# isarandi/metrabs

Hardware: NVIDIA H100
Metric: crops/sec (higher is better)
Workload: dtype bf16

## Files before the change

metrabs_b200/csrc/tc_fmb.cuh:

```cuda
#pragma once
#include "tc_gemm.cuh"

namespace mtb {

constexpr int FMB_NC = 128;
constexpr int FMB_BOX_H = TC_TILE_H + 2;
constexpr int FMB_BOX_BYTES = TC_TILE_W * FMB_BOX_H * TC_BK * 2;
constexpr int FMB_W_BYTES = FMB_NC * TC_BK * 2;
constexpr int FMB_A2_BYTES = TC_BM * FMB_NC * 2;

template <int BN2>
struct FmbSmem {
  static constexpr int kchunks = BN2 == 128 ? 2 : 1;
  static constexpr int stages = BN2 == 128 ? 4 : 8;
  static constexpr int ring_off = 3 * kchunks * FMB_BOX_BYTES;
  static constexpr int a2_off = ring_off + stages * FMB_W_BYTES;
  static constexpr int bar_off = a2_off + FMB_A2_BYTES;
  static constexpr int smem_bytes = bar_off + 256 + 1024 ;
};

struct FmbParams {
  TcConvParams g;
  const float* bias1;
  int Cexp, nch, has_res;
};

template <typename T, int BN2>
__global__ void __launch_bounds__(TC_THREADS, 1)
fmb_kernel(const __grid_constant__ CUtensorMap tmA, const __grid_constant__ CUtensorMap tmW1, const __grid_constant__ CUtensorMap tmW2,
           const FmbParams p) {
  using L = FmbSmem<BN2>;
  constexpr int STAGES = L::stages, KCH = L::kchunks, NUM_KB = 9 * KCH;
  extern __shared__ uint8_t tc_smem_raw[];
  uint8_t* smem = (uint8_t*)(((uintptr_t)tc_smem_raw + 1023) & ~(uintptr_t)1023);
  uint64_t* full = (uint64_t*)(smem + L::bar_off);
  uint64_t* empty = full + STAGES;
  uint64_t* box_full = empty + STAGES;
  uint64_t* box_empty = box_full + 1;
  const TcConvParams& g = p.g;

  const int warp = threadIdx.x >> 5, lane = threadIdx.x & 31;
  if (threadIdx.x == TC_CONSUMER_WARPS * 32) {
    tma_prefetch_desc(&tmA);
    tma_prefetch_desc(&tmW1);
    tma_prefetch_desc(&tmW2);
    for (int i = 0; i < STAGES; ++i) {
      mbar_init(&full[i], 1);
      mbar_init(&empty[i], TC_CONSUMER_WARPS);
    }
    mbar_init(box_full, 1);
    mbar_init(box_empty, TC_CONSUMER_WARPS);
    fence_barrier_init();
  }
  __syncthreads();

  if (warp == TC_CONSUMER_WARPS) {
    if (lane == 0) {
      int it = 0, n = 0;
      for (int t = blockIdx.x; t < g.m_tiles; t += gridDim.x, ++n) {
        mbar_wait(box_empty, (n & 1) ^ 1);
        mbar_expect_tx(box_full, 3 * KCH * FMB_BOX_BYTES);
#pragma unroll
        for (int kc = 0; kc < KCH; ++kc) tma_load_tap_boxes(smem + 3 * kc * FMB_BOX_BYTES, FMB_BOX_BYTES, &tmA, box_full, g, t, kc);
        for (int c = 0; c < p.nch; ++c) {
          for (int kb = 0; kb < NUM_KB + 2; ++kb, ++it) {
            const int s = it % STAGES;
            mbar_wait(&empty[s], ((it / STAGES) & 1) ^ 1);
            uint8_t* st = smem + L::ring_off + s * FMB_W_BYTES;
            if (kb < NUM_KB) {
              const int tap = kb / KCH, kc = kb - tap * KCH;
              mbar_expect_tx(&full[s], FMB_W_BYTES);
              tma_load_2d(st, &tmW1, &full[s], tap * g.Cin + kc * TC_BK, c * FMB_NC);
            } else {
              mbar_expect_tx(&full[s], BN2 * TC_BK * 2);
              tma_load_2d(st, &tmW2, &full[s], c * FMB_NC + (kb - NUM_KB) * TC_BK, 0);
            }
          }
        }
      }
    }
    return;
  }
  const int wg = warp >> 2;
  const uint32_t boxes = smem_u32(smem) + wg * 64 * 128, ring = smem_u32(smem + L::ring_off), a2 = smem_u32(smem + L::a2_off);
  const int r0 = wg * 64 + (warp & 3) * 16 + (lane >> 2);
  typedef typename Pair16<T>::type T2;
  const T* __restrict__ res = (const T*)g.res;
  T* __restrict__ out = (T*)g.out;
  int it = 0, n = 0;
  for (int t = blockIdx.x; t < g.m_tiles; t += gridDim.x, ++n) {
    float acc2[BN2 / 2];
#pragma unroll
    for (int i = 0; i < BN2 / 2; ++i) acc2[i] = 0.f;
    mbar_wait(box_full, n & 1);
    for (int c = 0; c < p.nch; ++c) {
      float acc1[FMB_NC / 2];
#pragma unroll
      for (int i = 0; i < FMB_NC / 2; ++i) acc1[i] = 0.f;
      int prev = -1;
      for (int kb = 0; kb < NUM_KB; ++kb, ++it) {
        const int s = it % STAGES;
        mbar_wait(&full[s], (it / STAGES) & 1);
        const int tap = kb / KCH, kc = kb - tap * KCH, r = tap / 3, sx = tap - 3 * r;
        const uint32_t a = boxes + (uint32_t)(3 * kc + sx) * FMB_BOX_BYTES + (uint32_t)r * (TC_TILE_W * 128);
        const uint32_t b = ring + s * FMB_W_BYTES;
        wgmma_fence();
#pragma unroll
        for (int k = 0; k < TC_BK / 16; ++k)
          wgmma_16b<T, FMB_NC>(acc1, gmma_desc<128>(a + 32 * k), gmma_desc<128>(b + 32 * k), (uint32_t)(kb | k));
        wgmma_commit();
        wgmma_wait<1>();
        if (prev >= 0) {
          __syncwarp();
          if (lane == 0) mbar_arrive(&empty[prev]);
        }
        prev = s;
      }
      wgmma_wait<0>();
      wgmma_fence_regs<FMB_NC / 2>(acc1);
      __syncwarp();
      if (lane == 0) {
        mbar_arrive(&empty[prev]);
        if (c == p.nch - 1) mbar_arrive(box_empty);
      }
#pragma unroll
      for (int j = 0; j < FMB_NC / 8; ++j) {
        const int cc = 8 * j + 2 * (lane & 3);
        const int col = c * FMB_NC + cc;
        float2 bv = make_float2(0.f, 0.f);
        if (col < p.Cexp) bv = __ldg(reinterpret_cast<const float2*>(p.bias1 + col));
        const uint32_t sub = (uint32_t)(cc >> 6) * (TC_BM * 128), kc = (uint32_t)(cc & 63);
#pragma unroll
        for (int h = 0; h < 2; ++h) {
          const int r = r0 + 8 * h;
          T2 v = Pair16<T>::pack(0.f, 0.f);
          if (col < p.Cexp)
            v = Pair16<T>::pack(tc_act<ACT_SILU, T>(acc1[4 * j + 2 * h] + bv.x), tc_act<ACT_SILU, T>(acc1[4 * j + 2 * h + 1] + bv.y));
          const uint32_t off = sub + (uint32_t)r * 128 + ((((kc >> 3) ^ (uint32_t)(r & 7))) << 4) + (kc & 7) * 2;
          *reinterpret_cast<T2*>(smem + L::a2_off + off) = v;
        }
      }
      fence_proxy_async();
      wg_sync(wg);
      {
        const int s0 = it % STAGES, s1 = (it + 1) % STAGES;
        mbar_wait(&full[s0], (it / STAGES) & 1);
        mbar_wait(&full[s1], ((it + 1) / STAGES) & 1);
        wgmma_fence();
#pragma unroll
        for (int k = 0; k < FMB_NC / 16; ++k) {
          const uint32_t sub = (uint32_t)(k >> 2), ko = (uint32_t)(k & 3) * 32;
          const uint32_t b = ring + (sub ? s1 : s0) * FMB_W_BYTES;
          wgmma_16b<T, BN2>(acc2, gmma_desc<128>(a2 + sub * (TC_BM * 128) + wg * 64 * 128 + ko), gmma_desc<128>(b + ko), (uint32_t)(c | k));
        }
        wgmma_commit();
        wgmma_wait<0>();
        wgmma_fence_regs<BN2 / 2>(acc2);
        __syncwarp();
        if (lane == 0) {
          mbar_arrive(&empty[s0]);
          mbar_arrive(&empty[s1]);
        }
        it += 2;
      }
    }
    const int c0 = 2 * (lane & 3);
#pragma unroll
    for (int h = 0; h < 2; ++h) {
      size_t off;
      if (!tile_row_offset(1, t, r0 + 8 * h, g.M, g.Cout, g.tiles_w, g.tiles_h, g.Hout, g.Wout, off)) continue;
#pragma unroll
      for (int j = 0; j < BN2 / 8; ++j) {
        const int cidx = c0 + 8 * j;
        if (cidx >= g.Cout) break;
        const float2 bv = __ldg(reinterpret_cast<const float2*>(g.bias + cidx));
        float o0 = acc2[4 * j + 2 * h] + bv.x, o1 = acc2[4 * j + 2 * h + 1] + bv.y;
        if (p.has_res) {
          const float2 rv = Pair16<T>::unpack(*reinterpret_cast<const T2*>(res + off + cidx));
          o0 += rv.x;
          o1 += rv.y;
        }
        *reinterpret_cast<T2*>(out + off + cidx) = Pair16<T>::pack(o0, o1);
      }
    }
  }
}

struct FmbWeights {
  bool ready = false;
  const TcWeights* w1 = nullptr;
  const TcWeights* w2 = nullptr;
  int Cin = 0, Cexp = 0, Cout = 0, bn2 = 0;
  mutable TmapCache maps;
};

inline bool fmb_shape_ok(int cin, int cexp, int cout) {
  return cin % 16 == 0 && cin >= 16 && cin <= 96 && cout == cin && cexp % 16 == 0 && cexp >= 32 && cexp <= 512;
}

inline void fmb_prepare(FmbWeights& f, const TcWeights& w1, const TcWeights& w2) {
  f.ready = false;
  if (!fmb_shape_ok(w1.Cin, w1.Cout, w2.Cout) || w2.Cin != w1.Cout || w1.taps != 9) return;
  f.w1 = &w1; f.w2 = &w2;
  f.Cin = w1.Cin; f.Cexp = w1.Cout; f.Cout = w2.Cout;
  f.bn2 = tc_pick_bn(f.Cout);
  f.ready = true;
}

template <typename T>
inline const char* fmb_launch(const FmbWeights& f, const void* in, void* out, int B, int H, int W, int pad_t, int pad_l, bool has_res,
                              cudaStream_t st) {
  if (!f.ready) return "fused FusedMBConv block not prepared";
  FmbParams q;
  TcConvParams& g = q.g;
  g.res = in; g.bias = f.w2->d_bias; g.out = out;
  g.mode = 1;
  g.Hin = H; g.Win = W; g.Hout = H; g.Wout = W;
  g.Cin = f.Cin; g.Cout = f.Cout;
  g.taps = 9; g.S = 3; g.stride = 1; g.dil = 1; g.pad_t = pad_t; g.pad_l = pad_l;
  g.kchunks = (f.Cin + TC_BK - 1) / TC_BK;
  g.tiles_w = (W + TC_TILE_W - 1) / TC_TILE_W;
  g.tiles_h = (H + TC_TILE_H - 1) / TC_TILE_H;
  g.M = B * H * W;
  q.bias1 = f.w1->d_bias;
  q.Cexp = f.Cexp;
  q.nch = (f.Cexp + FMB_NC - 1) / FMB_NC;
  q.has_res = has_res ? 1 : 0;
  const CUtensorMap* m = nullptr;
  const char* e = f.maps.get(&m, [&](CUtensorMap* c) {
    const CUtensorMapSwizzle sw = CU_TENSOR_MAP_SWIZZLE_128B;
    const char* r = make_tmap_nhwc<T>(&c[0], in, B, H, W, f.Cin, TC_BK, TC_TILE_W, FMB_BOX_H, 1, 1, sw);
    if (!r) r = make_tmap_2d<T>(&c[1], f.w1->d_w, f.Cexp, (uint64_t)9 * f.Cin, FMB_NC, TC_BK, sw);
    return r ? r : make_tmap_2d<T>(&c[2], f.w2->d_w, f.Cout, f.Cexp, f.bn2, TC_BK, sw);
  }, in, f.w1->d_w, f.w2->d_w, B, H, W, f.Cin, f.Cexp, f.Cout, f.bn2);
  if (e) return e;
  g.m_tiles = B * g.tiles_w * g.tiles_h;
  const int grid = std::min(g.m_tiles, num_sms());
  return with_const<32, 64, 128>(f.bn2, "unsupported N tile", [&](auto bn2) {
    if (q.g.kchunks != FmbSmem<bn2>::kchunks) return "fmb_kernel: k-chunks do not match the output width";
    return launch_smem(fmb_kernel<T, bn2>, dim3(grid), dim3(TC_THREADS), FmbSmem<bn2>::smem_bytes, st, m[0], m[1], m[2], q);
  });
}

}
```

metrabs_b200/csrc/tc_gemm.cuh:

```cuda
#pragma once
#include <cuda.h>

#include <algorithm>
#include <cstdio>
#include <cstdlib>
#include <cstring>
#include <string>
#include <vector>

#include "common.cuh"
#include "conv_simt.cuh"
#include "decode.cuh"
#include "wgmma.cuh"

namespace mtb {

__device__ __forceinline__ uint32_t smem_u32(const void* p) { return (uint32_t)__cvta_generic_to_shared(p); }

__device__ __forceinline__ void mbar_init(uint64_t* bar, uint32_t count) {
  asm volatile("mbarrier.init.shared::cta.b64 [%0], %1;" ::"r"(smem_u32(bar)), "r"(count));
}
__device__ __forceinline__ void mbar_expect_tx(uint64_t* bar, uint32_t bytes) {
  asm volatile("mbarrier.arrive.expect_tx.shared::cta.b64 _, [%0], %1;" ::"r"(smem_u32(bar)), "r"(bytes) : "memory");
}
// ... 288 lines not shown
    st_shared_u4(p0, v);
    st_shared_u4(p1, w);
  }
  if (r < re) se_scale_chunk<T>(a + r * 128 + ((L ^ (r & 7)) << 4), s0, s1);
}
template <typename T>
__device__ __forceinline__ void se_scale_a_tile(uint32_t a, uint64_t* full, uint32_t ph, const SeRows& w, const float* __restrict__ s, int m0,
                                                int P, int Cin, int kb, int u) {
  const int L = u & 7, k = kb * TC_BK + 8 * L;
  if (k >= Cin || w.r1 <= w.r0) {
    mbar_wait(full, ph);
    return;
  }
  const float4* sa = reinterpret_cast<const float4*>(s + (size_t)w.ca * Cin + k);
  const float4* sb = reinterpret_cast<const float4*>(s + (size_t)w.cb * Cin + k);
  const float4 a0 = __ldg(sa), a1 = __ldg(sa + 1), b0 = __ldg(sb), b1 = __ldg(sb + 1);
  if (k + TC_BK < Cin) {
    prefetch_l1(sa + TC_BK / 4);
    prefetch_l1(sb + TC_BK / 4);
  }
  mbar_wait(full, ph);
  const int ra = min((w.ca + 1) * P - m0, w.r1);
  const int rb = max(min(w.cb * P - m0, w.r1), ra);
  se_scale_rows<T>(a, L, w.r0, ra, a0, a1);
#pragma unroll 1
  for (int r = ra; r < rb; ++r) {
    const float4* sr = reinterpret_cast<const float4*>(s + (size_t)((m0 + r) / P) * Cin + k);
    se_scale_chunk<T>(a + r * 128 + ((L ^ (r & 7)) << 4), __ldg(sr), __ldg(sr + 1));
  }
  se_scale_rows<T>(a, L, rb, w.r1, b0, b1);
}

template <typename T, int ACT, int RES, int BN, bool SE = false>
__global__ void __launch_bounds__(TCP_THREADS, 1)
tc_conv_kernel(const __grid_constant__ CUtensorMap tmA, const __grid_constant__ CUtensorMap tmB, const __grid_constant__ CUtensorMap tmO,
               const TcConvParams p, const float* __restrict__ a_scale) {
  using Ring = TcRing<BN>;
  constexpr int STAGES = Ring::stages;
  extern __shared__ uint8_t tc_smem_raw[];
  uint8_t* smem = (uint8_t*)(((uintptr_t)tc_smem_raw + 1023) & ~(uintptr_t)1023);
  uint64_t* full = (uint64_t*)(smem + Ring::bar_off);
  uint64_t* empty = full + STAGES;
  uint64_t* ready = empty + STAGES;
  uint64_t* landed = SE ? ready : full;

  const int wg = threadIdx.x >> 7, lane = threadIdx.x & 31;
  if (threadIdx.x == 0) {
    tma_prefetch_desc(&tmA);
    tma_prefetch_desc(&tmB);
    tma_prefetch_desc(&tmO);
    for (int i = 0; i < STAGES; ++i) {
      mbar_init(&full[i], 1);
      mbar_init(&empty[i], 4);
      if constexpr (SE) mbar_init(&ready[i], 3);
    }
    fence_barrier_init();
  }
  __syncthreads();

  const int tiles = p.m_tiles * p.n_tiles;
  const int num_kb = SE ? p.kchunks : p.taps * p.kchunks;
  if (wg == 0) {
    setmaxnreg_dec<SE ? 56 : 40>();
    if (threadIdx.x == 0) {
      int it = 0;
      for (int t = blockIdx.x; t < tiles; t += gridDim.x) {
        const int m_blk = t / p.n_tiles, n_blk = t - m_blk * p.n_tiles;
        for (int kb = 0; kb < num_kb; ++kb, ++it) {
          const int s = it % STAGES;
          mbar_wait(&empty[s], ((it / STAGES) & 1) ^ 1);
          uint8_t* sa = smem + s * Ring::stage_bytes;
          const int tap = kb / p.kchunks, kc = kb - tap * p.kchunks;
          mbar_expect_tx(&full[s], Ring::stage_bytes);
          tma_load_a_tile<TC_BK>(sa, &tmA, &full[s], p, m_blk, kb);
          tma_load_2d(sa + TC_A_BYTES, &tmB, &full[s], tap * p.Cin + kc * TC_BK, n_blk * BN);
        }
      }
    } else if constexpr (SE) {
      if (threadIdx.x >= 32) {
        const int u = threadIdx.x - 32, P = p.Hin * p.Win;
        int it = 0;
        for (int t = blockIdx.x; t < tiles; t += gridDim.x) {
          const int m0 = (t / p.n_tiles) * TC_BM;
          const SeRows w = se_rows(u, m0, p.M, P);
          for (int kb = 0; kb < num_kb; ++kb, ++it) {
            const int s = it % STAGES;
            se_scale_a_tile<T>(smem_u32(smem + s * Ring::stage_bytes), &full[s], (it / STAGES) & 1, w, a_scale, m0, P, p.Cin, kb, u);
            fence_proxy_async();
            __syncwarp();
            if (lane == 0) mbar_arrive(&ready[s]);
          }
        }
      }
    }
    return;
  }
  setmaxnreg_inc<SE ? 224 : 232>();
  const int c = wg - 1;
  for (int i = c, t = blockIdx.x + c * gridDim.x; t < tiles; i += 2, t += 2 * gridDim.x) {
    const int m_blk = t / p.n_tiles, n_blk = t - m_blk * p.n_tiles;
    float acc[BN];
#pragma unroll
    for (int q = 0; q < BN; ++q) acc[q] = 0.f;
    if (t != (int)blockIdx.x) named_bar_sync(1 + c);
    int it = i * num_kb, prev = -1;
    for (int kb = 0; kb < num_kb; ++kb, ++it) {
      const int s = it % STAGES;
      mbar_wait(&landed[s], (it / STAGES) & 1);
      const uint32_t a = smem_u32(smem + s * Ring::stage_bytes);
      const uint32_t b = smem_u32(smem + s * Ring::stage_bytes + TC_A_BYTES);
      wgmma_fence();
#pragma unroll
      for (int k = 0; k < TC_BK / 16; ++k) {
        const uint64_t db = gmma_desc<128>(b + 32 * k);
        wgmma_16b<T, BN>(acc, gmma_desc<128>(a + 32 * k), db, (uint32_t)(kb | k));
        wgmma_16b<T, BN>(acc + BN / 2, gmma_desc<128>(a + 64 * 128 + 32 * k), db, (uint32_t)(kb | k));
      }
      wgmma_commit();
      wgmma_wait<1>();
      if (prev >= 0) {
        __syncwarp();
        if (lane == 0) mbar_arrive(&empty[prev]);
      }
      prev = s;
    }
    wgmma_wait<0>();
    wgmma_fence_regs<BN>(acc);
    __syncwarp();
    if (lane == 0) mbar_arrive(&empty[prev]);
    if (t + (int)gridDim.x < tiles) named_bar_arrive(2 - c);
    tc_tile_epilogue<T, ACT, RES, BN>(acc, smem + Ring::out_off + c * Ring::out_bytes, &tmO, p, m_blk, n_blk, c);
  }
  if ((threadIdx.x & 127) == 0) bulk_wait();
}

template <int CK>
struct Tc3x3Smem {
  static constexpr int RB = CK * 2;
  static constexpr int w_tap_bytes = CK * RB;
  static constexpr int box_bytes = TC_TILE_W * (TC_TILE_H + 2) * RB;
  static constexpr int sets = CK == 32 ? 2 : 1;
  static constexpr int box_off = 9 * w_tap_bytes;
  static constexpr int out_bytes = TC_BM * CK * 2;
  static constexpr int out_off = box_off + 2 * sets * 3 * box_bytes;
  static constexpr int bar_off = out_off + 2 * out_bytes;
  static constexpr int smem_bytes = bar_off + 256  + 1024 ;
};

inline bool tc3x3s1_eligible(int R, int S, int stride, int dil, int cin, int cout, int act) {
  return R == 3 && S == 3 && stride == 1 && dil == 1 && cin <= 64 && cout <= 64 && cin % 8 == 0 && cout % 8 == 0 &&
         (act == ACT_SILU || act == ACT_RELU);
}
inline int tc3x3s1_width(int cin, int cout) { return std::max(cin, cout) <= 32 ? 32 : 64; }

template <typename T, int ACT, int RES, int CK>
__global__ void __launch_bounds__(TCP_THREADS, 1)
tc_conv3x3s1_kernel(const __grid_constant__ CUtensorMap tmA, const __grid_constant__ CUtensorMap tmB,
                    const __grid_constant__ CUtensorMap tmO, const TcConvParams p) {
  using L = Tc3x3Smem<CK>;
  constexpr int BN = CK, SETS = L::sets, RB = L::RB;
  extern __shared__ uint8_t tc_smem_raw[];
  uint8_t* smem = (uint8_t*)(((uintptr_t)tc_smem_raw + 1023) & ~(uintptr_t)1023);
  uint64_t* w_full = (uint64_t*)(smem + L::bar_off);
  uint64_t* box_full = w_full + 1;
  uint64_t* box_empty = box_full + 2 * SETS;

  const int wg = threadIdx.x >> 7, lane = threadIdx.x & 31;
  if (threadIdx.x == 0) {
    tma_prefetch_desc(&tmA);
    tma_prefetch_desc(&tmB);
    tma_prefetch_desc(&tmO);
    mbar_init(w_full, 1);
    for (int i = 0; i < 2 * SETS; ++i) {
      mbar_init(&box_full[i], 1);
      mbar_init(&box_empty[i], 4);
    }
    fence_barrier_init();
  }
  __syncthreads();

  const int tiles = p.m_tiles;
  if (wg == 0) {
    setmaxnreg_dec<40>();
    if (threadIdx.x == 0) {
      mbar_expect_tx(w_full, 9 * L::w_tap_bytes);
      for (int tap = 0; tap < 9; ++tap) tma_load_2d(smem + tap * L::w_tap_bytes, &tmB, w_full, tap * p.Cin, 0);
      int n = 0;
      for (int t = blockIdx.x; t < tiles; t += gridDim.x, ++n) {
        const int j = n >> 1, b = (n & 1) * SETS + j % SETS;
        mbar_wait(&box_empty[b], ((j / SETS) & 1) ^ 1);
        mbar_expect_tx(&box_full[b], 3 * L::box_bytes);
        tma_load_tap_boxes(smem + L::box_off + b * 3 * L::box_bytes, L::box_bytes, &tmA, &box_full[b], p, t, 0);
      }
    }
    return;
  }
  setmaxnreg_inc<232>();
  const int c = wg - 1;
  const uint32_t wts = smem_u32(smem);
  mbar_wait(w_full, 0);
  for (int j = 0, t = blockIdx.x + c * gridDim.x; t < tiles; ++j, t += 2 * gridDim.x) {
    const int b = c * SETS + j % SETS;
    float acc[BN];
#pragma unroll
    for (int q = 0; q < BN; ++q) acc[q] = 0.f;
    mbar_wait(&box_full[b], (j / SETS) & 1);
    const uint32_t box = smem_u32(smem + L::box_off + b * 3 * L::box_bytes);
    wgmma_fence();
#pragma unroll
    for (int tap = 0; tap < 9; ++tap) {
      const int r = tap / 3, s = tap - 3 * r;
      const uint32_t a = box + s * L::box_bytes + r * TC_TILE_W * RB, w = wts + tap * L::w_tap_bytes;
#pragma unroll
      for (int k = 0; k < CK / 16; ++k) {
        const uint64_t db = gmma_desc<RB>(w + 32 * k);
        wgmma_16b<T, BN>(acc, gmma_desc<RB>(a + 32 * k), db, (uint32_t)(tap | k));
        wgmma_16b<T, BN>(acc + BN / 2, gmma_desc<RB>(a + 64 * RB + 32 * k), db, (uint32_t)(tap | k));
      }
    }
    wgmma_commit();
    wgmma_wait<0>();
    wgmma_fence_regs<BN>(acc);
    __syncwarp();
    if (lane == 0) mbar_arrive(&box_empty[b]);
    tc_tile_epilogue<T, ACT, RES, BN>(acc, smem + L::out_off + c * L::out_bytes, &tmO, p, t, 0, c);
  }
  if ((threadIdx.x & 127) == 0) bulk_wait();
}

template <typename T>
__global__ void __launch_bounds__(256) se_scale_kernel(T* __restrict__ x, const float* __restrict__ s, int P, int C,
                                                       size_t total8) {
  typedef typename Pair16<T>::type T2;
  for (size_t i = (size_t)blockIdx.x * blockDim.x + threadIdx.x; i < total8; i += (size_t)gridDim.x * blockDim.x) {
    size_t e = i * 8;
    int c = (int)(e % C);
    int b = (int)(e / ((size_t)P * C));
    uint4 v = *reinterpret_cast<uint4*>(x + e);
    T2* v2 = reinterpret_cast<T2*>(&v);
    const float4 s0 = *reinterpret_cast<const float4*>(s + (size_t)b * C + c);
    const float4 s1 = *reinterpret_cast<const float4*>(s + (size_t)b * C + c + 4);
    const float sc[8] = {s0.x, s0.y, s0.z, s0.w, s1.x, s1.y, s1.z, s1.w};
#pragma unroll
    for (int k = 0; k < 4; ++k) {
      float2 f = Pair16<T>::unpack(v2[k]);
      v2[k] = Pair16<T>::pack(f.x * sc[2 * k], f.y * sc[2 * k + 1]);
    }
    *reinterpret_cast<uint4*>(x + e) = v;
  }
}

typedef CUresult (*tmap_encode_fn)(CUtensorMap*, CUtensorMapDataType, cuuint32_t, void*, const cuuint64_t*, const cuuint64_t*,
                                   const cuuint32_t*, const cuuint32_t*, CUtensorMapInterleave, CUtensorMapSwizzle,
                                   CUtensorMapL2promotion, CUtensorMapFloatOOBfill);

inline tmap_encode_fn get_tmap_encode() {
  static tmap_encode_fn fn = nullptr;
  if (!fn) {
    void* p = nullptr;
    cudaDriverEntryPointQueryResult q;
    if (cudaGetDriverEntryPoint("cuTensorMapEncodeTiled", &p, cudaEnableDefault, &q) == cudaSuccess && q == cudaDriverEntryPointSuccess)
      fn = (tmap_encode_fn)p;
  }
  return fn;
}

template <typename T>
constexpr CUtensorMapDataType tmap_dtype() {
  return std::is_same<T, float>::value    ? CU_TENSOR_MAP_DATA_TYPE_FLOAT32
         : std::is_same<T, __half>::value ? CU_TENSOR_MAP_DATA_TYPE_FLOAT16
                                          : CU_TENSOR_MAP_DATA_TYPE_BFLOAT16;
}

template <typename T>
inline const char* make_tmap(CUtensorMap* m, const void* ptr, int rank, const uint64_t* dims, const uint32_t* box, const uint32_t* estr,
                             CUtensorMapSwizzle swizzle) {
  tmap_encode_fn enc = get_tmap_encode();
  if (!enc) return "cuTensorMapEncodeTiled unavailable";
  cuuint64_t strides[3];
  for (int i = 1; i < rank; ++i) strides[i - 1] = (i == 1 ? sizeof(T) : strides[i - 2]) * dims[i - 1];
  CUresult r = enc(m, tmap_dtype<T>(), rank, const_cast<void*>(ptr), dims, strides, box, estr, CU_TENSOR_MAP_INTERLEAVE_NONE, swizzle,
                   CU_TENSOR_MAP_L2_PROMOTION_L2_256B, CU_TENSOR_MAP_FLOAT_OOB_FILL_NONE);
  return r == CUDA_SUCCESS ? nullptr : "cuTensorMapEncodeTiled failed";
}
template <typename T>
inline const char* make_tmap_2d(CUtensorMap* m, const void* ptr, uint64_t rows, uint64_t cols, uint32_t box_rows, uint32_t box_cols,
                             CUtensorMapSwizzle swizzle) {
  const uint64_t dims[2] = {cols, rows};
  const uint32_t box[2] = {box_cols, box_rows}, estr[2] = {1, 1};
  return make_tmap<T>(m, ptr, 2, dims, box, estr, swizzle);
}
template <typename T>
inline const char* make_tmap_nhwc(CUtensorMap* m, const void* ptr, uint64_t B, uint64_t H, uint64_t W, uint64_t C, uint32_t box_c,
                             uint32_t box_w, uint32_t box_h, uint32_t box_b, uint32_t stride, CUtensorMapSwizzle swizzle) {
  const uint64_t dims[4] = {C, W, H, B};
  const uint32_t box[4] = {box_c, box_w * stride, box_h * stride, box_b}, estr[4] = {1, stride, stride, 1};
  return make_tmap<T>(m, ptr, 4, dims, box, estr, swizzle);
}

struct TmapCache {
  static constexpr int kEntries = 16, kKeyWords = 14;
  struct Entry {
    uint64_t key[kKeyWords];
    CUtensorMap map[3];
  };
  std::vector<Entry> entries;
  size_t replaced = 0;

  template <typename Encode, typename... K>
  const char* get(const CUtensorMap** maps, Encode&& encode, K... key) {
    static_assert(sizeof...(K) <= kKeyWords, "TmapCache key too long");
    Entry n = {};
    int i = 0;
    ((n.key[i++] = key_word(key)), ...);
    for (const Entry& e : entries)
      if (std::equal(e.key, e.key + kKeyWords, n.key)) {
        *maps = e.map;
        return nullptr;
      }
    if (const char* err = encode(n.map)) return err;
    Entry& slot = entries.size() < kEntries ? entries.emplace_back(n) : (entries[replaced++ % kEntries] = n);
    *maps = slot.map;
    return nullptr;
  }
  template <typename X>
  static uint64_t key_word(X x) {
    if constexpr (std::is_pointer<X>::value) return (uint64_t)(uintptr_t)x;
    else return (uint64_t)x;
  }
};

inline const char* upload_dev(std::vector<void*>& allocs, void** dev, const void* host, size_t bytes) {
  cudaError_t e = cudaMalloc(dev, bytes);
  if (e == cudaSuccess) {
    allocs.push_back(*dev);
    e = cudaMemcpy(*dev, host, bytes, cudaMemcpyHostToDevice);
  }
  return e == cudaSuccess ? nullptr : cudaGetErrorString(e);
}

struct TcWeights {
  bool ready = false;
  void* d_w = nullptr;
  float* d_bias = nullptr;
  int Cout = 0, Cin = 0, taps = 1, S = 1;
  int n_real = 0;
  mutable TmapCache maps;
};

inline bool tc_eligible(bool is_conv, bool depthwise, bool small_io, int k, int stride, int cin, int cout) {
  if (!is_conv || depthwise || small_io) return false;
  if (cin % 8 != 0 || cout % 8 != 0) return false;
  return (stride == 1 || stride == 2) && (k == 1 || k == 3);
}

inline __nv_bfloat16 host_bf16(float f) {
  uint32_t u;
  memcpy(&u, &f, 4);
  uint32_t lsb = (u >> 16) & 1u;
  u += 0x7FFFu + lsb;
  uint16_t h = (uint16_t)(u >> 16);
  __nv_bfloat16 out;
  memcpy(&out, &h, 2);
  return out;
}

inline __half host_f16(float f) { return __float2half_rn(f); }
template <typename T>
inline T host_16b(float f) {
  if constexpr (std::is_same<T, __half>::value) return host_f16(f);
  else return host_bf16(f);
}

template <typename T>
inline const char* tc_prepare_weights(TcWeights& w, const float* wk, const float* bias, int K, int cout, int R, int S, int cin,
                                      std::vector<void*>& allocs) {
  std::vector<T> t((size_t)K * cout);
  for (int k = 0; k < K; ++k)
    for (int n = 0; n < cout; ++n) t[(size_t)n * K + k] = host_16b<T>(wk[(size_t)k * cout + n]);
  const char* e = upload_dev(allocs, &w.d_w, t.data(), t.size() * sizeof(T));
  if (!e) e = upload_dev(allocs, (void**)&w.d_bias, bias, (size_t)cout * 4);
  if (e) return e;
  w.Cout = cout; w.Cin = cin; w.taps = R * S; w.S = S;
  w.ready = true;
  return nullptr;
}

inline int tc_pick_bn(int cout) { return cout <= 32 ? 32 : cout <= 64 ? 64 : 128; }
inline bool tc_se_in_gemm(int cout) { return cout <= 256; }

template <typename T>
inline const char* tc_conv_launch(const TcWeights& w, const ConvParams& p, bool res_first, cudaStream_t st) {
  TcConvParams q;
  q.res = p.res; q.bias = w.d_bias; q.out = p.out;
  q.mode = (p.R == 1 && p.stride == 1) ? 0 : 1;
  q.Hin = p.Hin; q.Win = p.Win;
  q.Cout = p.Cout; q.Cin = p.Cin;
  q.taps = w.taps; q.S = w.S; q.stride = p.stride; q.dil = p.dil;
  q.kchunks = (p.Cin + TC_BK - 1) / TC_BK;
  q.Hout = p.Hout; q.Wout = p.Wout; q.pad_t = p.pad_t; q.pad_l = p.pad_l;
  q.tiles_w = (p.Wout + TC_TILE_W - 1) / TC_TILE_W;
  q.tiles_h = (p.Hout + TC_TILE_H - 1) / TC_TILE_H;
  q.M = p.B * p.Hout * p.Wout;
  if (p.a_scale && (q.mode != 0 || !tc_se_in_gemm(p.Cout)))
    return "squeeze-excitation scale outside the 1x1 projections tc_conv_kernel scales (tc_se_in_gemm)";
  const bool s1 = tc3x3s1_eligible(p.R, p.S, p.stride, p.dil, p.Cin, p.Cout, p.act);
  const int bn = s1 ? tc3x3s1_width(p.Cin, p.Cout) : tc_pick_bn(p.Cout);
  q.m_tiles = q.mode == 0 ? (q.M + TC_BM - 1) / TC_BM : p.B * q.tiles_w * q.tiles_h;
  q.n_tiles = (p.Cout + bn - 1) / bn;
  const CUtensorMap* m = nullptr;
  const char* e = w.maps.get(&m, [&](CUtensorMap* c) {
    const CUtensorMapSwizzle sw = CU_TENSOR_MAP_SWIZZLE_128B;
    const uint32_t slab = (uint32_t)std::min(bn, 64);
    const CUtensorMapSwizzle out_sw = slab == 64 ? sw : CU_TENSOR_MAP_SWIZZLE_64B;
    const char* r;
    if (s1) {
      r = make_tmap_nhwc<T>(&c[0], p.in, p.B, p.Hin, p.Win, p.Cin, bn, TC_TILE_W, TC_TILE_H + 2, 1, 1, out_sw);
      if (!r) r = make_tmap_2d<T>(&c[1], w.d_w, p.Cout, (uint64_t)w.taps * p.Cin, bn, bn, out_sw);
    } else {
      r = q.mode == 0 ? make_tmap_2d<T>(&c[0], p.in, q.M, p.Cin, TC_BM, TC_BK, sw)
                      : make_tmap_nhwc<T>(&c[0], p.in, p.B, p.Hin, p.Win, p.Cin, TC_BK, TC_TILE_W, TC_TILE_H, 1, p.stride, sw);
      if (!r) r = make_tmap_2d<T>(&c[1], w.d_w, p.Cout, (uint64_t)w.taps * p.Cin, bn, TC_BK, sw);
    }
    if (!r)
      r = q.mode == 0 ? make_tmap_2d<T>(&c[2], p.out, q.M, p.Cout, TC_BM, slab, out_sw)
                      : make_tmap_nhwc<T>(&c[2], p.out, p.B, p.Hout, p.Wout, p.Cout, slab, TC_TILE_W, TC_TILE_H, 1, 1, out_sw);
    return r;
  }, p.in, p.out, w.d_w, p.B, p.Hin, p.Win, p.Cin, p.Hout, p.Wout, p.Cout, w.taps, p.stride, bn, s1);
  if (e) return e;
  const dim3 grid(std::min(q.m_tiles * q.n_tiles, num_sms()));
  const int res_mode = p.res ? (res_first ? 2 : 1) : 0;
  if (s1)
    return with_const<ACT_SILU, ACT_RELU>(p.act, "unsupported activation in tc_conv3x3s1_kernel", [&](auto act) {
      return with_const<0, 1, 2>(res_mode, "unsupported residual mode", [&](auto res) {
        return with_const<32, 64>(bn, "unsupported width of tc_conv3x3s1_kernel", [&](auto ck) {
          return launch_smem(tc_conv3x3s1_kernel<T, act, res, ck>, grid, dim3(TCP_THREADS), Tc3x3Smem<ck>::smem_bytes, st, m[0], m[1], m[2],
                             q);
        });
      });
    });
  if (p.a_scale)
    return with_const<ACT_NONE>(p.act, "unsupported activation with a squeeze-excitation scale", [&](auto act) {
      return with_const<0, 1>(res_mode, "unsupported residual mode with a squeeze-excitation scale", [&](auto res) {
        return with_const<32, 64, 128>(bn, "unsupported N tile", [&](auto bn_) {
          return launch_smem(tc_conv_kernel<T, act, res, bn_, true>, grid, dim3(TCP_THREADS), TcRing<bn_>::smem_bytes, st, m[0], m[1], m[2],
                             q, p.a_scale);
        });
      });
    });
  return with_const<ACT_NONE, ACT_SILU, ACT_RELU, ACT_HSWISH>(p.act, "unsupported activation in the tensor-core epilogue", [&](auto act) {
    return with_const<0, 1, 2>(res_mode, "unsupported residual mode", [&](auto res) {
      return with_const<32, 64, 128>(bn, "unsupported N tile", [&](auto bn_) {
        return launch_smem(tc_conv_kernel<T, act, res, bn_>, grid, dim3(TCP_THREADS), TcRing<bn_>::smem_bytes, st, m[0], m[1], m[2], q,
                           (const float*)nullptr);
      });
    });
  });
}

template <typename T>
inline const char* tc_se_scale_launch(void* x, const float* s, int B, int P, int C, cudaStream_t st) {
  size_t total8 = (size_t)B * P * C / 8;
  launch_k(se_scale_kernel<T>, dim3(grid_for(total8, 256)), dim3(256), 0, st, (T*)x, s, P, C, total8);
  cudaError_t e = cudaGetLastError();
  return e == cudaSuccess ? nullptr : cudaGetErrorString(e);
}

struct TcHeadParams {
  float4* states;
  const float* bias;
  int B, P, W, n_out, C;
  int bnp;
  int cpt;
  int npt;
  int m_tiles;
  int kblocks;
};
constexpr int TCH_STAGES = 2;
constexpr int TCH_STAGE_BYTES = TC_A_BYTES + 256 * TC_BK * 2;
constexpr int TCH_STG_OFF = TCH_STAGES * TCH_STAGE_BYTES;
constexpr int TCH_BAR_OFF = TCH_STG_OFF + 128 * 256 * 4;
constexpr int TCH_SMEM_BYTES = TCH_BAR_OFF + 64 + 1024 ;

__device__ __forceinline__ uint32_t tch_stg(int row, int col) {
  return (uint32_t)(row * 256 + ((((col >> 2) ^ (row & 7))) << 2) + (col & 3)) * 4u;
}

template <typename T>
__global__ void __launch_bounds__(TC_THREADS, 1)
tc_head_kernel(const __grid_constant__ CUtensorMap tmW, const __grid_constant__ CUtensorMap tmF, const TcHeadParams p) {
  extern __shared__ uint8_t tc_smem_raw[];
  uint8_t* smem = (uint8_t*)(((uintptr_t)tc_smem_raw + 1023) & ~(uintptr_t)1023);
  uint64_t* full = (uint64_t*)(smem + TCH_BAR_OFF);
  uint64_t* empty = full + TCH_STAGES;
  float* stg = (float*)(smem + TCH_STG_OFF);

  const int warp = threadIdx.x >> 5, lane = threadIdx.x & 31;
  if (threadIdx.x == TC_CONSUMER_WARPS * 32) {
    tma_prefetch_desc(&tmW);
    tma_prefetch_desc(&tmF);
    for (int i = 0; i < TCH_STAGES; ++i) {
      mbar_init(&full[i], 1);
      mbar_init(&empty[i], TC_CONSUMER_WARPS);
    }
    fence_barrier_init();
  }
  __syncthreads();

  const int g = blockIdx.x / p.m_tiles, m_blk = blockIdx.x - g * p.m_tiles;
  const int n_kb = p.npt * p.kblocks;
  if (warp == TC_CONSUMER_WARPS) {
    if (lane == 0) {
      const uint32_t stage_tx = TC_A_BYTES + (uint32_t)p.bnp * TC_BK * 2;
      for (int i = 0; i < n_kb; ++i) {
        const int s = i % TCH_STAGES, pt = i / p.kblocks, kb = i - pt * p.kblocks;
        mbar_wait(&empty[s], ((i / TCH_STAGES) & 1) ^ 1);
        uint8_t* sa = smem + s * TCH_STAGE_BYTES;
        const int row0 = p.cpt > 0 ? g * p.bnp : g * p.P + pt * p.bnp;
        mbar_expect_tx(&full[s], stage_tx);
        tma_load_2d(sa, &tmW, &full[s], kb * TC_BK, m_blk * TC_BM);
        tma_load_2d(sa + TC_A_BYTES, &tmF, &full[s], kb * TC_BK, row0);
      }
    }
    return;
  }
  const int wg = warp >> 2, tid = threadIdx.x & 127;
  const int row = wg * 64 + tid;
  const int n = m_blk * TC_BM + row;
  const bool owner = tid < 64;
  const bool nvalid = owner && n < p.n_out;
  const float bias_n = nvalid ? p.bias[n] : 0.f;
  constexpr float L2E = 1.4426950408889634f;
  int crop = p.cpt > 0 ? g * p.cpt : g;
  int pix = 0, x = 0, y = 0;
  float m = -INFINITY, mL = -INFINITY, s_ = 0.f, sx = 0.f, sy = 0.f;
  int i = 0;
  for (int pt = 0; pt < p.npt; ++pt) {
    float acc[128];
#pragma unroll
    for (int k = 0; k < 128; ++k) acc[k] = 0.f;
    int prev = -1;
    for (int kb = 0; kb < p.kblocks; ++kb, ++i) {
      const int s = i % TCH_STAGES;
      mbar_wait(&full[s], (i / TCH_STAGES) & 1);
      const uint32_t a = smem_u32(smem + s * TCH_STAGE_BYTES) + wg * 64 * 128;
      const uint32_t b = smem_u32(smem + s * TCH_STAGE_BYTES + TC_A_BYTES);
      wgmma_fence();
#pragma unroll
      for (int k = 0; k < TC_BK / 16; ++k) wgmma_16b<T, 256>(acc, gmma_desc<128>(a + 32 * k), gmma_desc<128>(b + 32 * k), (uint32_t)(kb | k));
      wgmma_commit();
      wgmma_wait<1>();
      if (prev >= 0) {
        __syncwarp();
        if (lane == 0) mbar_arrive(&empty[prev]);
      }
      prev = s;
    }
    wgmma_wait<0>();
    wgmma_fence_regs<128>(acc);
    __syncwarp();
    if (lane == 0) mbar_arrive(&empty[prev]);
    {
      const int fr = wg * 64 + (warp & 3) * 16 + (lane >> 2), fc = 2 * (lane & 3);
#pragma unroll
      for (int j = 0; j < 32; ++j) {
        *reinterpret_cast<float2*>((uint8_t*)stg + tch_stg(fr, fc + 8 * j)) = make_float2(acc[4 * j], acc[4 * j + 1]);
        *reinterpret_cast<float2*>((uint8_t*)stg + tch_stg(fr + 8, fc + 8 * j)) = make_float2(acc[4 * j + 2], acc[4 * j + 3]);
      }
    }
    wg_sync(wg);
    if (owner) {
      for (int c0 = 0; c0 < p.bnp; c0 += 16) {
        float v[16];
#pragma unroll
        for (int q = 0; q < 4; ++q) {
          const float4 f = *reinterpret_cast<const float4*>((const uint8_t*)stg + tch_stg(row, c0 + 4 * q));
          v[4 * q] = f.x; v[4 * q + 1] = f.y; v[4 * q + 2] = f.z; v[4 * q + 3] = f.w;
        }
        if (pix + 16 <= p.P) {
          float vm = v[0];
#pragma unroll
          for (int q = 1; q < 16; ++q) vm = fmaxf(vm, v[q]);
          vm += bias_n;
          if (vm > m) {
            const float mL_new = vm * L2E;
            float f = ex2_fast(mL - mL_new);
            s_ *= f; sx *= f; sy *= f;
            m = vm;
            mL = mL_new;
          }
          const float cL = fmaf(bias_n, L2E, -mL);
#pragma unroll
          for (int q = 0; q < 16; ++q) {
            float e = ex2_fast(fmaf(v[q], L2E, cL));
            s_ += e;
            sx = fmaf(e, (float)x, sx);
            sy = fmaf(e, (float)y, sy);
            if (++x == p.W) { x = 0; ++y; }
          }
          pix += 16;
          if (pix == p.P) {
            if (nvalid && crop < p.B) p.states[(size_t)crop * p.n_out + n] = make_float4(m, s_, sx, sy);
            ++crop; pix = 0; x = 0; y = 0;
            m = -INFINITY; mL = -INFINITY; s_ = 0.f; sx = 0.f; sy = 0.f;
          }
        } else {
#pragma unroll
// ... 116 lines not shown
```

Measured before the change: 6878.

## Stage fused MBConv epilogue in smem and store via TMA; cache biases in smem

The fused expand/project kernel now writes its final output tile into the shared A2 buffer with swizzle and issues TMA 4D stores, replacing per-thread scattered global stores. Both bias vectors are preloaded into shared memory, and bias and residual loads are batched ahead of use. For single-k-chunk configurations the two warpgroups take turns writing the intermediate through named barriers. These changes aim to cut global-store and load latency in the epilogue, at the cost of extra barriers and bulk-store waits before the A2 buffer is reused.

```diff
diff --git a/metrabs_b200/csrc/tc_fmb.cuh b/metrabs_b200/csrc/tc_fmb.cuh
--- a/metrabs_b200/csrc/tc_fmb.cuh
+++ b/metrabs_b200/csrc/tc_fmb.cuh
@@ -8,6 +8,8 @@
 constexpr int FMB_BOX_BYTES = TC_TILE_W * FMB_BOX_H * TC_BK * 2;
 constexpr int FMB_W_BYTES = FMB_NC * TC_BK * 2;
 constexpr int FMB_A2_BYTES = TC_BM * FMB_NC * 2;
+constexpr int FMB_EB = 8;
+constexpr int FMB_BAR_WG0_DONE = 3, FMB_BAR_WG1_DONE = 4;
 
 template <int BN2>
 struct FmbSmem {
@@ -16,7 +18,8 @@
   static constexpr int ring_off = 3 * kchunks * FMB_BOX_BYTES;
   static constexpr int a2_off = ring_off + stages * FMB_W_BYTES;
   static constexpr int bar_off = a2_off + FMB_A2_BYTES;
-  static constexpr int smem_bytes = bar_off + 256 + 1024 ;
+  static constexpr int bias_off = bar_off + 256;
+  static constexpr int smem_bytes = bias_off + (4 * FMB_NC + BN2) * 4 + 1024 ;
 };
 
 struct FmbParams {
@@ -28,22 +31,29 @@
 template <typename T, int BN2>
 __global__ void __launch_bounds__(TC_THREADS, 1)
 fmb_kernel(const __grid_constant__ CUtensorMap tmA, const __grid_constant__ CUtensorMap tmW1, const __grid_constant__ CUtensorMap tmW2,
-           const FmbParams p) {
+           const __grid_constant__ CUtensorMap tmO, const FmbParams p) {
   using L = FmbSmem<BN2>;
   constexpr int STAGES = L::stages, KCH = L::kchunks, NUM_KB = 9 * KCH;
+  constexpr bool TURNS = KCH == 1;
   extern __shared__ uint8_t tc_smem_raw[];
-  uint8_t* smem = (uint8_t*)(((uintptr_t)tc_smem_raw + 1023) & ~(uintptr_t)1023);
+  uint8_t* smem = tc_smem_raw + ((1024u - (smem_u32(tc_smem_raw) & 1023u)) & 1023u);
   uint64_t* full = (uint64_t*)(smem + L::bar_off);
   uint64_t* empty = full + STAGES;
   uint64_t* box_full = empty + STAGES;
   uint64_t* box_empty = box_full + 1;
   const TcConvParams& g = p.g;
+  float* bias_s = (float*)(smem + L::bias_off);
+  for (int i = threadIdx.x; i < 4 * FMB_NC + BN2; i += blockDim.x) {
+    const int k = i - 4 * FMB_NC;
+    bias_s[i] = k < 0 ? (i < p.Cexp ? p.bias1[i] : 0.f) : (k < g.Cout ? g.bias[k] : 0.f);
+  }
 
   const int warp = threadIdx.x >> 5, lane = threadIdx.x & 31;
   if (threadIdx.x == TC_CONSUMER_WARPS * 32) {
     tma_prefetch_desc(&tmA);
     tma_prefetch_desc(&tmW1);
     tma_prefetch_desc(&tmW2);
+    tma_prefetch_desc(&tmO);
     for (int i = 0; i < STAGES; ++i) {
       mbar_init(&full[i], 1);
       mbar_init(&empty[i], TC_CONSUMER_WARPS);
@@ -86,13 +96,16 @@
   const int r0 = wg * 64 + (warp & 3) * 16 + (lane >> 2);
   typedef typename Pair16<T>::type T2;
   const T* __restrict__ res = (const T*)g.res;
-  T* __restrict__ out = (T*)g.out;
   int it = 0, n = 0;
   for (int t = blockIdx.x; t < g.m_tiles; t += gridDim.x, ++n) {
     float acc2[BN2 / 2];
 #pragma unroll
     for (int i = 0; i < BN2 / 2; ++i) acc2[i] = 0.f;
     mbar_wait(box_full, n & 1);
+    if (n > 0) {
+      if ((threadIdx.x & 127) == 0) bulk_wait_read();
+      wg_sync(wg);
+    }
     for (int c = 0; c < p.nch; ++c) {
       float acc1[FMB_NC / 2];
 #pragma unroll
@@ -123,25 +136,38 @@
         mbar_arrive(&empty[prev]);
         if (c == p.nch - 1) mbar_arrive(box_empty);
       }
-#pragma unroll
-      for (int j = 0; j < FMB_NC / 8; ++j) {
-        const int cc = 8 * j + 2 * (lane & 3);
-        const int col = c * FMB_NC + cc;
-        float2 bv = make_float2(0.f, 0.f);
-        if (col < p.Cexp) bv = __ldg(reinterpret_cast<const float2*>(p.bias1 + col));
-        const uint32_t sub = (uint32_t)(cc >> 6) * (TC_BM * 128), kc = (uint32_t)(cc & 63);
-#pragma unroll
-        for (int h = 0; h < 2; ++h) {
-          const int r = r0 + 8 * h;
-          T2 v = Pair16<T>::pack(0.f, 0.f);
-          if (col < p.Cexp)
-            v = Pair16<T>::pack(tc_act<ACT_SILU, T>(acc1[4 * j + 2 * h] + bv.x), tc_act<ACT_SILU, T>(acc1[4 * j + 2 * h + 1] + bv.y));
-          const uint32_t off = sub + (uint32_t)r * 128 + ((((kc >> 3) ^ (uint32_t)(r & 7))) << 4) + (kc & 7) * 2;
-          *reinterpret_cast<T2*>(smem + L::a2_off + off) = v;
+      if constexpr (TURNS) {
+        if (wg == 1) named_bar_sync(FMB_BAR_WG0_DONE);
+        else if (c > 0 || n > 0) named_bar_sync(FMB_BAR_WG1_DONE);
+      }
+#pragma unroll
+      for (int j0 = 0; j0 < FMB_NC / 8; j0 += FMB_EB) {
+        float2 bv[FMB_EB];
+#pragma unroll
+        for (int jj = 0; jj < FMB_EB; ++jj) bv[jj] = *reinterpret_cast<const float2*>(bias_s + c * FMB_NC + 8 * (j0 + jj) + 2 * (lane & 3));
+#pragma unroll
+        for (int j = j0; j < j0 + FMB_EB; ++j) {
+          const int cc = 8 * j + 2 * (lane & 3);
+          const int col = c * FMB_NC + cc;
+          const uint32_t sub = (uint32_t)(cc >> 6) * (TC_BM * 128), kc = (uint32_t)(cc & 63);
+#pragma unroll
+          for (int h = 0; h < 2; ++h) {
+            const int r = r0 + 8 * h;
+            T2 v = Pair16<T>::pack(0.f, 0.f);
+            if (col < p.Cexp)
+              v = Pair16<T>::pack(tc_act<ACT_SILU, T>(acc1[4 * j + 2 * h] + bv[j - j0].x),
+                                  tc_act<ACT_SILU, T>(acc1[4 * j + 2 * h + 1] + bv[j - j0].y));
+            const uint32_t off = sub + (uint32_t)r * 128 + ((((kc >> 3) ^ (uint32_t)(r & 7))) << 4) + (kc & 7) * 2;
+            *reinterpret_cast<T2*>(smem + L::a2_off + off) = v;
+          }
         }
       }
       fence_proxy_async();
       wg_sync(wg);
+      if constexpr (TURNS) {
+        if (wg == 0) named_bar_arrive(FMB_BAR_WG0_DONE);
+        else if (c < p.nch - 1 || t + (int)gridDim.x < g.m_tiles) named_bar_arrive(FMB_BAR_WG1_DONE);
+      }
       {
         const int s0 = it % STAGES, s1 = (it + 1) % STAGES;
         mbar_wait(&full[s0], (it / STAGES) & 1);
@@ -167,23 +193,49 @@
     const int c0 = 2 * (lane & 3);
 #pragma unroll
     for (int h = 0; h < 2; ++h) {
+      const int r = r0 + 8 * h;
       size_t off;
-      if (!tile_row_offset(1, t, r0 + 8 * h, g.M, g.Cout, g.tiles_w, g.tiles_h, g.Hout, g.Wout, off)) continue;
-#pragma unroll
-      for (int j = 0; j < BN2 / 8; ++j) {
-        const int cidx = c0 + 8 * j;
-        if (cidx >= g.Cout) break;
-        const float2 bv = __ldg(reinterpret_cast<const float2*>(g.bias + cidx));
-        float o0 = acc2[4 * j + 2 * h] + bv.x, o1 = acc2[4 * j + 2 * h + 1] + bv.y;
+      if (!tile_row_offset(1, t, r, g.M, g.Cout, g.tiles_w, g.tiles_h, g.Hout, g.Wout, off)) continue;
+      constexpr int JB = BN2 == 128 ? 4 : BN2 / 8 < 8 ? BN2 / 8 : 8;
+#pragma unroll
+      for (int j0 = 0; j0 < BN2 / 8; j0 += JB) {
+        T2 rv2[JB];
+        float2 bv2[JB];
+#pragma unroll
+        for (int jj = 0; jj < JB; ++jj) bv2[jj] = *reinterpret_cast<const float2*>(bias_s + 4 * FMB_NC + c0 + 8 * (j0 + jj));
         if (p.has_res) {
-          const float2 rv = Pair16<T>::unpack(*reinterpret_cast<const T2*>(res + off + cidx));
-          o0 += rv.x;
-          o1 += rv.y;
-        }
-        *reinterpret_cast<T2*>(out + off + cidx) = Pair16<T>::pack(o0, o1);
-      }
-    }
-  }
+#pragma unroll
+          for (int jj = 0; jj < JB; ++jj)
+            if (c0 + 8 * (j0 + jj) < g.Cout) rv2[jj] = *reinterpret_cast<const T2*>(res + off + c0 + 8 * (j0 + jj));
+        }
+#pragma unroll
+        for (int j = j0; j < j0 + JB; ++j) {
+          const int cidx = c0 + 8 * j;
+          if (cidx >= g.Cout) break;
+          float o0 = acc2[4 * j + 2 * h] + bv2[j - j0].x, o1 = acc2[4 * j + 2 * h + 1] + bv2[j - j0].y;
+          if (p.has_res) {
+            const float2 rv = Pair16<T>::unpack(rv2[j - j0]);
+            o0 += rv.x;
+            o1 += rv.y;
+          }
+          const uint32_t sub = (uint32_t)(cidx >> 6) * (TC_BM * 128), kc = (uint32_t)(cidx & 63);
+          const uint32_t o = sub + (uint32_t)r * 128 + ((((kc >> 3) ^ (uint32_t)(r & 7))) << 4) + (kc & 7) * 2;
+          *reinterpret_cast<T2*>(smem + L::a2_off + o) = Pair16<T>::pack(o0, o1);
+        }
+      }
+    }
+    fence_proxy_async();
+    wg_sync(wg);
+    if ((threadIdx.x & 127) == 0) {
+      const int tw = t % g.tiles_w, th = (t / g.tiles_w) % g.tiles_h, b = t / (g.tiles_w * g.tiles_h);
+#pragma unroll
+      for (int sl = 0; sl < (BN2 + 63) / 64; ++sl)
+        if (sl * 64 < g.Cout)
+          tma_store_4d(&tmO, smem + L::a2_off + sl * (TC_BM * 128) + wg * 64 * 128, sl * 64, tw * TC_TILE_W, th * TC_TILE_H + wg * 4, b);
+      bulk_commit();
+    }
+  }
+  if ((threadIdx.x & 127) == 0) bulk_wait();
 }
 
 struct FmbWeights {
@@ -231,14 +283,15 @@
     const CUtensorMapSwizzle sw = CU_TENSOR_MAP_SWIZZLE_128B;
     const char* r = make_tmap_nhwc<T>(&c[0], in, B, H, W, f.Cin, TC_BK, TC_TILE_W, FMB_BOX_H, 1, 1, sw);
     if (!r) r = make_tmap_2d<T>(&c[1], f.w1->d_w, f.Cexp, (uint64_t)9 * f.Cin, FMB_NC, TC_BK, sw);
-    return r ? r : make_tmap_2d<T>(&c[2], f.w2->d_w, f.Cout, f.Cexp, f.bn2, TC_BK, sw);
-  }, in, f.w1->d_w, f.w2->d_w, B, H, W, f.Cin, f.Cexp, f.Cout, f.bn2);
+    if (!r) r = make_tmap_2d<T>(&c[2], f.w2->d_w, f.Cout, f.Cexp, f.bn2, TC_BK, sw);
+    return r ? r : make_tmap_nhwc<T>(&c[3], out, B, H, W, f.Cout, TC_BK, TC_TILE_W, TC_TILE_H / 2, 1, 1, sw);
+  }, in, out, f.w1->d_w, f.w2->d_w, B, H, W, f.Cin, f.Cexp, f.Cout, f.bn2);
   if (e) return e;
   g.m_tiles = B * g.tiles_w * g.tiles_h;
   const int grid = std::min(g.m_tiles, num_sms());
   return with_const<32, 64, 128>(f.bn2, "unsupported N tile", [&](auto bn2) {
     if (q.g.kchunks != FmbSmem<bn2>::kchunks) return "fmb_kernel: k-chunks do not match the output width";
-    return launch_smem(fmb_kernel<T, bn2>, dim3(grid), dim3(TC_THREADS), FmbSmem<bn2>::smem_bytes, st, m[0], m[1], m[2], q);
+    return launch_smem(fmb_kernel<T, bn2>, dim3(grid), dim3(TC_THREADS), FmbSmem<bn2>::smem_bytes, st, m[0], m[1], m[2], m[3], q);
   });
 }
 
diff --git a/metrabs_b200/csrc/tc_gemm.cuh b/metrabs_b200/csrc/tc_gemm.cuh
--- a/metrabs_b200/csrc/tc_gemm.cuh
+++ b/metrabs_b200/csrc/tc_gemm.cuh
@@ -614,7 +614,7 @@
   static constexpr int kEntries = 16, kKeyWords = 14;
   struct Entry {
     uint64_t key[kKeyWords];
-    CUtensorMap map[3];
+    CUtensorMap map[4];
   };
   std::vector<Entry> entries;
   size_t replaced = 0;
```

New measurement: 7010 (median of 6 runs). 1.9% higher.
